# wwyuan2023/VITS

Hardware: AMD Instinct MI355X
Metric: 22.05 kHz audio samples/sec/GPU (infer RTF) + train utt/sec at 1/2/4/8 MI355X (higher is better)
Workload: dtype fp32; 1 GPU; SynthesizerTrn.infer_p2 batch=16 Tx=100 Ty=500 (configs/base.json, 16 kHz, hop 192) per GPU; global_batch=16, seq_len=500, parallelism=single GPU, graph=False

## Files before the change

### vits_amd/csrc/resblock_f32p.hip

```cpp
#include <type_traits>

#include "conv1d_impl.h"

namespace {

using vits_conv::fast_sigmoid;
using vits_conv::fast_tanh;
using vits_conv::split3_bf16x4;

constexpr int RP_GROUP = 3;
struct RpGroup {
  vits_resblock_pair_desc d[RP_GROUP];
  int n;
  int batch;
  int bn;
};

typedef __bf16 bf16x8 __attribute__((ext_vector_type(8)));
typedef __bf16 bf16x4 __attribute__((ext_vector_type(4)));
typedef __bf16 bf16x2 __attribute__((ext_vector_type(2)));
typedef float f32x4v __attribute__((ext_vector_type(4)));

template <int MODE>
struct RpT {
  typedef float xt;
  typedef __bf16 lt;
  static constexpr int NPL = 3;
};
template <>
struct RpT<1> {
  typedef __bf16 xt;
  typedef __bf16 lt;
  static constexpr int NPL = 1;
};
template <>
struct RpT<2> {
  typedef _Float16 xt;
  typedef _Float16 lt;
  static constexpr int NPL = 1;
};
__host__ __device__ constexpr int rp_npl(int mode) { return mode == 0 ? 3 : 1; }

__host__ __device__ constexpr int rp_ng(int C) { return C <= 64 ? 256 : 128; }
__host__ __device__ constexpr int rp_threads(int C) { return C == 256 ? 512 : 256; }
#ifndef VITS_RP_KC32
#define VITS_RP_KC32 32
#endif
__host__ __device__ constexpr int rp_kc(int C, int mode = 0) {
  return C == 256 ? 64 : C == 32 ? VITS_RP_KC32 : 16;
}
__host__ __device__ inline int rp_xcols(int NG, int k, int dil) {
  return ((NG + (k - 1) * dil + 3 + 3) >> 2) << 2;
}
__host__ __device__ inline int rp_lds_bytes(int C, int k, int dil, int mode = 0) {
  const int NG = rp_ng(C), npl = rp_npl(mode);
  const int nbuf = rp_kc(C, mode) < C ? 2 : 1;
  const int xs = nbuf * npl * rp_xcols(NG, k, dil) * (rp_kc(C, mode) + 4);
  const int gsz = npl * (NG + 16) * (C / 2 + 8);
  return 4 * 2 * C + 2 * (xs > gsz ? xs : gsz) + 64;
}
__host__ __device__ constexpr int rp_occ(int C, int) { return C == 256 ? 1 : 2; }

__device__ __forceinline__ float rp_gate(float a, float b) {
#pragma clang fp contract(off)
  return fast_tanh(a) * fast_sigmoid(b);
}

__device__ __forceinline__ float rp_max(float a, float b) {
  float r;
  asm("v_max_f32 %0, %1, %2" : "=v"(r) : "v"(a), "v"(b));
  return r;
}

template <int C, int MODE = 0, bool MEAN = false>
__global__ __launch_bounds__(rp_threads(C), rp_occ(C, MODE)) void resblock_f32p_kernel(
    const RpGroup G) {
  typedef std::integral_constant<bool, true> edge_t;
  typedef std::integral_constant<bool, false> interior_t;
  typedef typename RpT<MODE>::xt xt;
  typedef typename RpT<MODE>::lt lt;
  constexpr int NPL = RpT<MODE>::NPL;
  typedef lt lt8 __attribute__((ext_vector_type(8)));
  typedef lt lt4 __attribute__((ext_vector_type(4)));
  typedef lt lt2 __attribute__((ext_vector_type(2)));
  typedef xt xt4 __attribute__((ext_vector_type(4)));
  constexpr int H = C / 2;
  constexpr int NT = rp_threads(C);
  constexpr int WAVES_M = C >= 64 ? C / 64 : 1;
  constexpr int WAVES_N = NT / 64 / WAVES_M;
  constexpr int NG = 64 * WAVES_N;
  static_assert(NG == rp_ng(C), "tile columns");
  constexpr int TM = C >= 64 ? 2 : 1, TN = 2;
  constexpr int KC = rp_kc(C, MODE);
  constexpr int KCP = KC + 4;
  constexpr int GP = H + 8;
  constexpr int GPL = (NG + 16) * GP;
  constexpr int S1 = C / 16, S2 = H / 16;
  constexpr int NU = ((KC / 4) * ((NG + 102) / 4) + NT - 1) / NT;
  typedef lt8 av_t;
  constexpr int NB = NPL == 3 ? TN : 1;

  const int gi = MEAN ? 0 : (int)blockIdx.z / G.batch;
  const int b = (int)blockIdx.z - gi * G.batch;
  const int Tn = G.d[gi].t_len;
  const int L = G.d[gi].lengths ? min(Tn, (int)G.d[gi].lengths[b]) : Tn;
  const int BN = MEAN ? G.bn : NG - (G.d[gi].k - 1);
  const int n0 = blockIdx.x * BN;
  if (n0 >= Tn) return;
  if (G.d[gi].lengths && G.d[gi].len_skip > 0 && n0 >= L + G.d[gi].len_skip) return;

  extern __shared__ float smem[];
  float* const erow = smem;
  lt* const reg = reinterpret_cast<lt*>(smem + 2 * C);

  const int tid = threadIdx.x;
  const int lane = tid & 63;
  const int wid = __builtin_amdgcn_readfirstlane(tid >> 6);
  const int wn = (wid % WAVES_N) * 64;
  const int wm = (wid / WAVES_N) * 64;
  const int l32 = lane & 31;
  const int lhi = lane >> 5;

  float msum[TM][TN][MEAN ? 16 : 1];

#pragma unroll 1
  for (int br = 0; br < (MEAN ? G.n : 1); ++br) {
    const vits_resblock_pair_desc& p = G.d[MEAN ? br : gi];
    const int k = p.k;
    const int dil = p.dil;
    const int p1 = (k - 1) * dil / 2;
    const int p2 = (k - 1) / 2;
    const int tw0 = n0 - p2 - p1;
    const int xstart = tw0 & ~3;
    const int xcols = rp_xcols(NG, k, dil);
    const bool interior = xstart >= 0 && xstart + xcols <= Tn && n0 - p2 + NG <= L;
    if (MEAN && br > 0) __syncthreads();

    {
      const float* cond = p.cond ? p.cond + (int64_t)b * p.cond_bstride : nullptr;
      for (int r = tid; r < 2 * C; r += NT) {
        float e = 0.f;
        if (r < C) {
          const int idx = (r & 1) ? H + (r >> 1) : (r >> 1);
          if (p.b1) e = p.b1[idx];
          if (cond) e += cond[idx];
        } else if (p.b2) {
          e = p.b2[r - C];
        }
        erow[r] = e;
      }
    }

    f32x16 acc[TM][TN];
#pragma unroll
    for (int i = 0; i < TM; ++i)
#pragma unroll
      for (int j = 0; j < TN; ++j)
#pragma unroll
        for (int r = 0; r < 16; ++r) acc[i][j][r] = 0.f;

    auto mma = [&](av_t (*a)[TM], const av_t* bh, const av_t* bm, const av_t* bl) {
#pragma unroll
      for (int mi = 0; mi < TM; ++mi)
#pragma unroll
        for (int ni = 0; ni < TN; ++ni) {
          f32x16 c = acc[mi][ni];
          if constexpr (MODE == 0) {
            c = __builtin_amdgcn_mfma_f32_32x32x16_bf16(a[0][mi], bl[ni], c, 0, 0, 0);
            c = __builtin_amdgcn_mfma_f32_32x32x16_bf16(a[2][mi], bh[ni], c, 0, 0, 0);
            c = __builtin_amdgcn_mfma_f32_32x32x16_bf16(a[1][mi], bm[ni], c, 0, 0, 0);
            c = __builtin_amdgcn_mfma_f32_32x32x16_bf16(a[0][mi], bm[ni], c, 0, 0, 0);
            c = __builtin_amdgcn_mfma_f32_32x32x16_bf16(a[1][mi], bh[ni], c, 0, 0, 0);
            c = __builtin_amdgcn_mfma_f32_32x32x16_bf16(a[0][mi], bh[ni], c, 0, 0, 0);
          } else if constexpr (MODE == 1) {
            c = __builtin_amdgcn_mfma_f32_32x32x16_bf16(a[0][mi], bh[ni], c, 0, 0, 0);
          } else {
            c = __builtin_amdgcn_mfma_f32_32x32x16_f16(a[0][mi], bh[ni], c, 0, 0, 0);
          }
          acc[mi][ni] = c;
        }
    };
    auto loadA = [&](const lt* wl, int64_t wstep, int m_pad, int s, int total,
                     av_t (*a)[TM]) {
      const lt* wp = wl + (int64_t)(s < total ? s : total - 1) * wstep;
#pragma unroll
      for (int q = 0; q < NPL; ++q)
#pragma unroll
        for (int mi = 0; mi < TM; ++mi)
          a[q][mi] = *reinterpret_cast<const av_t*>(wp + ((int64_t)q * m_pad + mi * 32) * 8);
    };

    av_t a0[NPL][TM], a1[NPL][TM];
    av_t bh0[TN], bm0[NB], bl0[NB], bh1[TN], bm1[NB], bl1[NB];

    const xt* xb = reinterpret_cast<const xt*>(p.x) + (int64_t)b * p.x_bstride;
    {
      const int xsh = tw0 - xstart;
      const int nunits = (KC / 4) * (xcols >> 2);
      const int xpl = xcols * KCP;
      lt* const xbuf0 = reg;
      lt* const xbuf1 = reg + NPL * xpl;
      const float slope = p.in_slope;
      xt4 xr[NU][4];
      uint32_t xoff[NU];
      bool xok[NU];
#pragma unroll
      for (int q = 0; q < NU; ++q) {
        const int u = tid + NT * q;
        const int tt = xstart + 4 * (u / (KC / 4));
        xok[q] = u < nunits && tt >= 0 && tt < Tn;
        xoff[q] = xok[q] ? 4 * (u % (KC / 4)) * p.x_cstride + tt : 0;
      }
      auto gload = [&](int ch) __attribute__((always_inline)) {
        const xt* base = xb + (int64_t)ch * KC * p.x_cstride;
#pragma unroll
        for (int q = 0; q < NU; ++q) {
          if (q * NT < nunits) {
#pragma unroll
            for (int i = 0; i < 4; ++i)
              xr[q][i] = *reinterpret_cast<const xt4*>(base + (int64_t)i * p.x_cstride + xoff[q]);
          }
        }
      };
      const bool xfast = interior && slope > 0.f && slope < 1.f;
      auto lstore_as = [&](lt* xs, auto edge) __attribute__((always_inline)) {
#pragma unroll
        for (int q = 0; q < NU; ++q) {
          const int u = tid + NT * q;
          if (q * NT < nunits && u < nunits) {
            f32x4v v[4];
#pragma unroll
            for (int i = 0; i < 4; ++i)
#pragma unroll
              for (int e = 0; e < 4; ++e) {
                float t = (float)xr[q][i][e];
                if constexpr (decltype(edge)::value) {
                  t = t < 0.f ? t * slope : t;
                  v[i][e] = xok[q] ? t : 0.f;
                } else {
                  v[i][e] = rp_max(t, t * slope);
                }
              }
            lt* xh = xs + 4 * (u / (KC / 4)) * KCP + 4 * (u % (KC / 4));
#pragma unroll
            for (int e = 0; e < 4; ++e) {
              const f32x4v w = {v[0][e], v[1][e], v[2][e], v[3][e]};
              if constexpr (NPL == 3) {
                bf16x4 h4, m4, l4;
                split3_bf16x4(w, h4, m4, l4);
                *reinterpret_cast<bf16x4*>(xh + e * KCP) = h4;
                *reinterpret_cast<bf16x4*>(xh + xpl + e * KCP) = m4;
                *reinterpret_cast<bf16x4*>(xh + 2 * xpl + e * KCP) = l4;
              } else {
                lt4 w4;
#pragma unroll
                for (int i = 0; i < 4; ++i) w4[i] = (lt)w[i];
                *reinterpret_cast<lt4*>(xh + e * KCP) = w4;
              }
            }
          }
        }
      };
      auto lstore = [&](lt* xs) __attribute__((always_inline)) {
        if (xfast)
          lstore_as(xs, interior_t());
        else
          lstore_as(xs, edge_t());
      };
      auto loadB = [&](const lt* xs, int j, int g, av_t* bh, av_t* bm, av_t* bl) {
        const int P4 = xpl / 4;
#pragma unroll
        for (int ni = 0; ni < TN; ++ni) {
          const lt4* xp = reinterpret_cast<const lt4*>(
              xs + (wn + ni * 32 + l32 + j * dil + xsh) * KCP + 16 * g + 8 * lhi);
          bh[ni] = __builtin_shufflevector(xp[0], xp[1], 0, 1, 2, 3, 4, 5, 6, 7);
          if constexpr (NPL == 3) {
            bm[ni] = __builtin_shufflevector(xp[P4], xp[P4 + 1], 0, 1, 2, 3, 4, 5, 6, 7);
            bl[ni] = __builtin_shufflevector(xp[2 * P4], xp[2 * P4 + 1], 0, 1, 2, 3, 4, 5, 6, 7);
          }
        }
      };
      const lt* wl = reinterpret_cast<const lt*>(p.w1) +
                     ((int64_t)(lhi * NPL) * p.m_pad1 + wm + l32) * 8;
      const int64_t wstep = (int64_t)16 * NPL * p.m_pad1;
      const int total = S1 * k;
      const int nst = (KC / 16) * k;
      loadA(wl, wstep, p.m_pad1, 0, total, a0);
      gload(0);
      lstore(xbuf0);
      __syncthreads();
      for (int ch = 0; ch < C / KC; ++ch) {
        const bool more = ch + 1 < C / KC;
        if (more) gload(ch + 1);
        const lt* xs = (ch & 1) ? xbuf1 : xbuf0;
        const int s0 = ch * nst;
        int j = 0, g = 0;
        auto next = [&]() {
          if (++j == k) {
            j = 0;
            ++g;
          }
        };
        loadB(xs, 0, 0, bh0, bm0, bl0);
        int st = 0;
        for (; st + 2 <= nst; st += 2) {
          next();
          loadA(wl, wstep, p.m_pad1, s0 + st + 1, total, a1);
          loadB(xs, j, g, bh1, bm1, bl1);
          __builtin_amdgcn_sched_barrier(0);
          mma(a0, bh0, bm0, bl0);
          __builtin_amdgcn_sched_barrier(0);
          next();
          loadA(wl, wstep, p.m_pad1, s0 + st + 2, total, a0);
          if (st + 2 < nst) loadB(xs, j, g, bh0, bm0, bl0);
          __builtin_amdgcn_sched_barrier(0);
          mma(a1, bh1, bm1, bl1);
          __builtin_amdgcn_sched_barrier(0);
        }
        if (st < nst) {
          loadA(wl, wstep, p.m_pad1, s0 + nst, total, a1);
          __builtin_amdgcn_sched_barrier(0);
          mma(a0, bh0, bm0, bl0);
#pragma unroll
          for (int q = 0; q < NPL; ++q)
#pragma unroll
            for (int mi = 0; mi < TM; ++mi) a0[q][mi] = a1[q][mi];
        }
        if (more) lstore((ch & 1) ? xbuf0 : xbuf1);
        __syncthreads();
      }
    }

    lt* const gs = reg;
    auto gate = [&](auto edge) __attribute__((always_inline)) {
#pragma unroll
      for (int mi = 0; mi < TM; ++mi) {
        f32x4v er[4];
#pragma unroll
        for (int g = 0; g < 4; ++g)
          er[g] = *reinterpret_cast<const f32x4v*>(erow + wm + mi * 32 + 4 * lhi + 8 * g);
#pragma unroll
        for (int ni = 0; ni < TN; ++ni) {
          const int col = wn + ni * 32 + l32;
          const int t = n0 - p2 + col;
          const bool in = t >= 0 && t < L;
#pragma unroll
          for (int r = 0; r < 16; r += 4) {
            const int row = wm + mi * 32 + 4 * lhi + 8 * (r >> 2);
            const f32x4v e = er[r >> 2];
            float g0 = rp_gate(acc[mi][ni][r] + e[0], acc[mi][ni][r + 1] + e[1]);
            float g1 = rp_gate(acc[mi][ni][r + 2] + e[2], acc[mi][ni][r + 3] + e[3]);
            if constexpr (decltype(edge)::value) {
              g0 = in ? g0 : 0.f;
              g1 = in ? g1 : 0.f;
            }
            lt* gp = gs + col * GP + (row >> 1);
            if constexpr (NPL == 3) {
              const f32x4v w = {g0, g1, 0.f, 0.f};
              bf16x4 h4, m4, l4;
              split3_bf16x4(w, h4, m4, l4);
              *reinterpret_cast<bf16x2*>(gp) = __builtin_shufflevector(h4, h4, 0, 1);
              *reinterpret_cast<bf16x2*>(gp + GPL) = __builtin_shufflevector(m4, m4, 0, 1);
              *reinterpret_cast<bf16x2*>(gp + 2 * GPL) = __builtin_shufflevector(l4, l4, 0, 1);
            } else {
              lt2 v2;
              v2[0] = (lt)g0;
              v2[1] = (lt)g1;
              *reinterpret_cast<lt2*>(gp) = v2;
            }
          }
#pragma unroll
          for (int r = 0; r < 16; ++r) acc[mi][ni][r] = 0.f;
        }
      }
    };
    if (interior)
      gate(interior_t());
    else
      gate(edge_t());
    for (int i = tid; i < NPL * 16 * H; i += NT) {
      const int pl = i / (16 * H);
      const int e = i - pl * 16 * H;
      gs[pl * GPL + (NG + e / H) * GP + e % H] = (lt)0.f;
    }
    __syncthreads();

    {
      const lt* wl = reinterpret_cast<const lt*>(p.w2) +
                     ((int64_t)(lhi * NPL) * p.m_pad2 + wm + l32) * 8;
      const int64_t wstep = (int64_t)16 * NPL * p.m_pad2;
      const int total = S2 * k;
      const lt* gl = gs + (wn + l32) * GP + 8 * lhi;
      int j = 0, g = 0;
      auto loadB = [&](av_t* bh, av_t* bm, av_t* bl) {
        const lt* x = gl + j * GP + 16 * g;
#pragma unroll
        for (int ni = 0; ni < TN; ++ni) {
          bh[ni] = *reinterpret_cast<const av_t*>(x + ni * 32 * GP);
          if constexpr (NPL == 3) {
            bm[ni] = *reinterpret_cast<const av_t*>(x + ni * 32 * GP + GPL);
            bl[ni] = *reinterpret_cast<const av_t*>(x + ni * 32 * GP + 2 * GPL);
          }
        }
        if (++j == k) {
          j = 0;
          ++g;
        }
      };
      loadA(wl, wstep, p.m_pad2, 0, total, a0);
      loadB(bh0, bm0, bl0);
      int s = 0;
      for (; s + 2 <= total; s += 2) {
        loadA(wl, wstep, p.m_pad2, s + 1, total, a1);
        loadB(bh1, bm1, bl1);
        __builtin_amdgcn_sched_barrier(0);
        mma(a0, bh0, bm0, bl0);
        __builtin_amdgcn_sched_barrier(0);
        loadA(wl, wstep, p.m_pad2, s + 2, total, a0);
        if (s + 2 < total) loadB(bh0, bm0, bl0);
        __builtin_amdgcn_sched_barrier(0);
        mma(a1, bh1, bm1, bl1);
        __builtin_amdgcn_sched_barrier(0);
      }
      if (s < total) mma(a0, bh0, bm0, bl0);
    }

    xt* const yb = reinterpret_cast<xt*>(p.y) + (int64_t)b * p.y_bstride;
    const bool accum = !MEAN && p.accumulate;
    const float div = MEAN ? (float)G.n : p.post_div;
    const bool last = !MEAN || br == G.n - 1;
    auto epilogue = [&](auto edge) __attribute__((always_inline)) {
#pragma unroll
      for (int mi = 0; mi < TM; ++mi) {
        const xt* const xrow = xb + (int64_t)(wm + mi * 32) * p.x_cstride;
        xt* const yrow = yb + (int64_t)(wm + mi * 32) * p.y_cstride;
        f32x4v e2[4];
#pragma unroll
        for (int g = 0; g < 4; ++g)
          e2[g] = *reinterpret_cast<const f32x4v*>(erow + C + wm + mi * 32 + 4 * lhi + 8 * g);
#pragma unroll
        for (int ni = 0; ni < TN; ++ni) {
          const int col = wn + ni * 32 + l32;
          const int t = n0 + col;
          const bool st = decltype(edge)::value ? col < BN && t < Tn : col < BN;
          const int tc = st ? t : 0;
          const uint32_t xv = (uint32_t)(4 * lhi * p.x_cstride + tc) * (uint32_t)sizeof(xt);
          const uint32_t yv = (uint32_t)(4 * lhi * p.y_cstride + tc) * (uint32_t)sizeof(xt);
          auto xat = [&](int r) __attribute__((always_inline)) -> const xt& {
            const xt* row = xrow + (int64_t)((r & 3) + 8 * (r >> 2)) * p.x_cstride;
            return *reinterpret_cast<const xt*>(reinterpret_cast<const char*>(row) + xv);
          };
          auto yat = [&](int r) __attribute__((always_inline)) -> xt& {
            xt* row = yrow + (int64_t)((r & 3) + 8 * (r >> 2)) * p.y_cstride;
            return *reinterpret_cast<xt*>(reinterpret_cast<char*>(row) + yv);
          };
          float o[16];
#pragma unroll
          for (int r = 0; r < 16; ++r) {
            const float rv = (float)xat(r);
            const float v = acc[mi][ni][r] + e2[r >> 2][r & 3];
            o[r] = rv + v;
          }
          if constexpr (MEAN) {
#pragma unroll
            for (int r = 0; r < 16; ++r) {
              o[r] = br == 0 ? o[r] : msum[mi][ni][r] + o[r];
              msum[mi][ni][r] = o[r];
            }
          }
          if (accum) {
#pragma unroll
            for (int r = 0; r < 16; ++r)
              o[r] = (float)yat(r) + o[r];
          }
          if (last) {
            if (div != 1.0f) {
#pragma unroll
              for (int r = 0; r < 16; ++r) o[r] = o[r] / div;
            }
            if (st) {
#pragma unroll
              for (int r = 0; r < 16; ++r) {
                if constexpr (decltype(edge)::value) o[r] = t < L ? o[r] : 0.f;
                yat(r) = (xt)o[r];
              }
            }
          }
        }
      }
    };
    if (interior)
      epilogue(interior_t());
    else
      epilogue(edge_t());
  }
}

template <int C, int MODE = 0, bool MEAN = false>
int rp_launch(const RpGroup& g, hipStream_t s) {
  int lds = 0, gx = 0;
  for (int i = 0; i < g.n; ++i) {
    const vits_resblock_pair_desc& d = g.d[i];
    const int l = rp_lds_bytes(C, d.k, d.dil, MODE);
    if (l > lds) lds = l;
    const int BN = MEAN ? g.bn : rp_ng(C) - (d.k - 1);
    const int x = (d.t_len + BN - 1) / BN;
    if (x > gx) gx = x;
  }
  if (lds > 160 * 1024) return VITS_E_UNSUP;
  hipLaunchKernelGGL((resblock_f32p_kernel<C, MODE, MEAN>),
                     dim3(gx, 1, MEAN ? g.batch : g.n * g.batch), dim3(rp_threads(C)), lds, s, g);
  return vits_launch_status();
}

int rp_check(const vits_resblock_pair_desc& d, int mode = 0) {
  VITS_CHECK_ARG(d.x && d.w1 && d.w2 && d.y);
  VITS_CHECK_ARG(reinterpret_cast<const void*>(d.y) != reinterpret_cast<const void*>(d.x));
  VITS_CHECK_SHAPE(d.channels == 32 || d.channels == 64 || d.channels == 128 ||
                   d.channels == 256);
  VITS_CHECK_SHAPE(d.k >= 1 && d.k <= 15 && (d.k & 1) == 1 && d.dil >= 1 && d.t_len > 0);
  VITS_CHECK_SHAPE((d.k - 1) * d.dil <= 96);
  VITS_CHECK_SHAPE(d.m_pad1 >= d.channels && d.m_pad2 >= d.channels && (d.m_pad1 & 3) == 0 &&
                   (d.m_pad2 & 3) == 0);
  VITS_CHECK_SHAPE(d.cin_pad1 >= d.channels && d.cin_pad2 >= d.channels / 2);
  VITS_CHECK_SHAPE((d.t_len & 3) == 0 && (d.x_cstride & 3) == 0 && (d.x_bstride & 3) == 0 &&
                   d.x_cstride >= d.t_len && d.y_cstride >= d.t_len &&
                   (reinterpret_cast<uintptr_t>(d.x) & (mode ? 7 : 15)) == 0);
  VITS_CHECK_SHAPE((int64_t)d.channels * d.x_cstride < (1LL << 31));
  VITS_CHECK_SHAPE((int64_t)d.channels * d.y_cstride < (1LL << 31));
  VITS_CHECK_SHAPE((reinterpret_cast<uintptr_t>(d.w1) & 15) == 0 &&
                   (reinterpret_cast<uintptr_t>(d.w2) & 15) == 0);
  return VITS_OK;
}

}

int vits_rp16_256(const vits_resblock_pair_desc* d, int n, int batch, int wdtype,
                  hipStream_t s) {
  if (!d || n < 1 || n > RP_GROUP || batch < 1) return VITS_E_ARG;
  if (wdtype != VITS_WDT_BF16 && wdtype != VITS_WDT_F16) return VITS_E_ARG;
  const int mode = wdtype == VITS_WDT_BF16 ? 1 : 2;
  RpGroup g;
  g.n = n;
  g.batch = batch;
  g.bn = 0;
  for (int i = 0; i < n; ++i) {
    const int rc = rp_check(d[i], mode);
    if (rc) return rc;
    if (d[i].channels != d[0].channels) return VITS_E_SHAPE;
    g.d[i] = d[i];
  }
  if (d[0].channels != 256) return VITS_E_SHAPE;
  return mode == 1 ? rp_launch<256, 1>(g, s) : rp_launch<256, 2>(g, s);
}

extern "C" int vits_resblock_pair_f32p_forward(const vits_resblock_pair_desc* d, int n, int batch,
                                               void* stream) {
  if (!d || n < 1 || n > RP_GROUP || batch < 1) return VITS_E_ARG;
  RpGroup g;
  g.n = n;
  g.batch = batch;
  g.bn = 0;
  for (int i = 0; i < n; ++i) {
    const int rc = rp_check(d[i]);
    if (rc) return rc;
    if (d[i].channels != d[0].channels) return VITS_E_SHAPE;
    g.d[i] = d[i];
  }
  hipStream_t s = as_stream(stream);
  int rc;
  if (d[0].channels == 32)
    rc = rp_launch<32>(g, s);
  else if (d[0].channels == 64)
    rc = rp_launch<64>(g, s);
  else if (d[0].channels == 128)
    rc = rp_launch<128>(g, s);
  else
    rc = rp_launch<256>(g, s);
  return count_ok(rc, VITS_CNT_RESBLOCK);
}

extern "C" int vits_resblock_pair_f32p_mean_forward(const vits_resblock_pair_desc* d, int n,
                                                    int batch, void* stream) {
  if (!d || n < 1 || n > RP_GROUP || batch < 1) return VITS_E_ARG;
  RpGroup g;
  g.n = n;
  g.batch = batch;
  int kmax = 1;
  for (int i = 0; i < n; ++i) {
    const int rc = rp_check(d[i]);
    if (rc) return rc;
    VITS_CHECK_SHAPE(d[i].channels == 32);
    VITS_CHECK_SHAPE(d[i].t_len == d[0].t_len && d[i].lengths == d[0].lengths &&
                     d[i].len_skip == d[0].len_skip && d[i].y == d[0].y &&
                     d[i].y_bstride == d[0].y_bstride && d[i].y_cstride == d[0].y_cstride);
    VITS_CHECK_ARG(reinterpret_cast<const void*>(d[0].y) != reinterpret_cast<const void*>(d[i].x));
    if (d[i].k > kmax) kmax = d[i].k;
    g.d[i] = d[i];
  }
  g.bn = rp_ng(32) - (kmax - 1);
  return count_ok(rp_launch<32, 0, true>(g, as_stream(stream)), VITS_CNT_RESBLOCK);
}
```

### vits_amd/ops.py

```python
from __future__ import annotations

import contextlib
import ctypes as C
import math
import threading
from dataclasses import dataclass, field
from fractions import Fraction
from typing import Optional

import numpy as np
import torch

from . import _lib
from ._lib import (ACT_NONE, WDT_BF16, WDT_F16, WDT_F32, WDT_F32P, WDT_F32S, ConvDesc, ConvOut, EPI_GATE, EPI_STORE,
                   ResblockPairDesc,
                   EPI_UPSAMPLE, TILE_128x128, TILE_32x256, TILE_64x128, TILE_64x256, TILE_ROWS,
                   check)



def _stream_ptr(device: torch.device) -> int:
    return torch.cuda.current_stream(device).cuda_stream


# ... 179 lines not shown
    m = (r.view(torch.int32) & mask).view(torch.float32)
    lo = r - m
    return torch.stack([h, m, lo], dim=-3).to(torch.bfloat16)


F32S_MIN_ROWS = 0


def _f32s_min_rows() -> int:
    return F32S_MIN_ROWS or (64 if SPLIT_W else 128)


def to_lowp(layer: PackedConv, wdtype: int = WDT_BF16, min_rows: Optional[int] = None) -> PackedConv:
    if layer.wdtype != WDT_F32 or wdtype == WDT_F32:
        return layer
    if wdtype == WDT_F32S:
        if layer.m < (_f32s_min_rows() if min_rows is None else min_rows):
            return layer
        kc = 16
        w32 = layer.w[:layer.cin]
        cin_pad = (layer.cin + kc - 1) // kc * kc
        k, m_pad = w32.shape[1], w32.shape[2]
        w = w32.new_zeros(cin_pad, k, m_pad)
        w[:layer.cin] = w32
        w = w.view(cin_pad // kc, kc // 8, 8, k, m_pad).permute(0, 3, 1, 4, 2).contiguous()
        if SPLIT_W:
            tile = _pick_tile_f32p(layer.m, layer.k)
            return PackedConv(split_planes(w), layer.bias, layer.cin, layer.m, layer.k,
                              layer.dil, layer.pad_left, layer.epi, tile,
                              _kc_f32p(cin_pad, layer.k, layer.dil, tile), up_u=layer.up_u,
                              up_pad=layer.up_pad, out_channels=layer.out_channels,
                              extra=layer.extra, wdtype=WDT_F32P)
        return PackedConv(w, layer.bias, layer.cin, layer.m, layer.k, layer.dil,
                          layer.pad_left, layer.epi, _pick_tile_f32s(layer.m, layer.k), kc,
                          up_u=layer.up_u, up_pad=layer.up_pad,
                          out_channels=layer.out_channels, extra=layer.extra, wdtype=wdtype)
    kc = 16
    w32 = layer.w[:layer.cin]
    cin_pad = (layer.cin + kc - 1) // kc * kc
    k, m_pad = w32.shape[1], w32.shape[2]
    w = w32.new_zeros(cin_pad, k, m_pad)
    w[:layer.cin] = w32
    w = w.view(cin_pad // kc, kc // 8, 8, k, m_pad).permute(0, 3, 1, 4, 2).contiguous()
    tile = _pick_tile_bf16(layer.m, layer.k)
    return PackedConv(w.to(_WDT_TORCH[wdtype]), layer.bias, layer.cin, layer.m, layer.k,
                      layer.dil, layer.pad_left, layer.epi, tile, kc, up_u=layer.up_u,
                      up_pad=layer.up_pad, out_channels=layer.out_channels, extra=layer.extra,
                      wdtype=wdtype)


LOWP_KCK = 512


def io16_kc(layer: PackedConv) -> int:
    bm, bn = TILE_ROWS[layer.tile], TILE_COLS[layer.tile]
    xrs = bn + (layer.k - 1) * layer.dil + 8
    xbudget = 6144 if bn <= 128 else 10240
    for kc in (64, 48, 32):
        if (kc * layer.k <= LOWP_KCK and layer.cin_pad % kc == 0
                and kc * layer.k * bm // 2 <= 6144 and kc * xrs <= xbudget):
            return kc
    return 16


def to_bf16(layer: PackedConv) -> PackedConv:
    return to_lowp(layer, WDT_BF16)


def pack_conv(weight: torch.Tensor, bias: Optional[torch.Tensor], *, dilation: int = 1,
              padding: Optional[int] = None, gate: bool = False) -> PackedConv:
    w = weight.detach().to(torch.float32)
    cout, cin, k = w.shape
    if padding is None:
        padding = (k * dilation - dilation) // 2
    if gate:
        assert cout % 2 == 0
        h = cout // 2
        rows = torch.stack([w[:h], w[h:]], dim=1).reshape(cout, cin, k)
        epi, outc = EPI_GATE, h
    else:
        rows, epi, outc = w, EPI_STORE, cout
    tile = _pick_tile(cout, k)
    packed, kc = _finish_pack(rows, k, tile, dilation)
    b = None if bias is None else bias.detach().to(torch.float32).contiguous()
    layer = PackedConv(packed, b, cin, cout, k, dilation, padding, epi, tile, kc,
                       out_channels=outc)
    return to_lowp(layer, PACK_PRECISION.wdtype)


def pack_conv_transpose(weight: torch.Tensor, bias: Optional[torch.Tensor], stride: int,
                        padding: int) -> PackedConv:
    w = weight.detach().to(torch.float32)
    cin, cout, K = w.shape
    u = stride
    assert K % u == 0, "polyphase lowering needs kernel_size % stride == 0"
    kp = K // u
    w4 = w.reshape(cin, cout, kp, u)
    rows = w4.flip(2).permute(1, 3, 0, 2).reshape(cout * u, cin, kp)
    tile = _pick_tile(cout * u, kp)
    packed, kc = _finish_pack(rows, kp, tile)
    b = None if bias is None else bias.detach().to(torch.float32).contiguous()
    layer = PackedConv(packed, b, cin, cout * u, kp, 1, kp - 1, EPI_UPSAMPLE, tile, kc,
                       up_u=u, up_pad=padding, out_channels=cout)
    return to_lowp(layer, PACK_PRECISION.wdtype)




def make_out(y: torch.Tensor, *, act: int = ACT_NONE, res: Optional[torch.Tensor] = None,
             res_scale: float = 1.0, accumulate: bool = False, post_div: float = 1.0,
             channel_offset: int = 0) -> ConvOut:
    o = ConvOut()
    o.y = y.data_ptr() + y.element_size() * channel_offset * y.stride(1)
    o.y_bstride = y.stride(0)
    o.y_cstride = y.stride(1)
    o.act = act
    if res is not None:
        o.res = res.data_ptr() + res.element_size() * channel_offset * res.stride(1)
        o.res_bstride = res.stride(0)
        o.res_cstride = res.stride(1)
    else:
        o.res = None
        o.res_bstride = 0
        o.res_cstride = 0
    o.res_scale = res_scale
    o.accumulate = 1 if accumulate else 0
    o.post_div = post_div
    return o


_LOWP_TORCH = {WDT_F16: torch.float16, WDT_BF16: torch.bfloat16}


class _LenSkip(threading.local):
    margin = 0


LEN_SKIP = _LenSkip()


@contextlib.contextmanager
def length_skip(margin: int = 64):
    old = LEN_SKIP.margin
    LEN_SKIP.margin = int(margin)
    try:
        yield
    finally:
        LEN_SKIP.margin = old


def make_desc(layer: PackedConv, x: torch.Tensor, out0: ConvOut, *, out1: Optional[ConvOut] = None,
              split: Optional[int] = None, tin: Optional[int] = None, n_out: Optional[int] = None,
              in_slope: float = 1.0, cond: Optional[torch.Tensor] = None, cond_offset: int = 0,
              lengths: Optional[torch.Tensor] = None, t_out: int = 0,
              x_channel_offset: int = 0, io16: bool = False) -> ConvDesc:
    if io16:
        assert layer.wdtype != WDT_F32 and x.dtype == _LOWP_TORCH[layer.wdtype]
    else:
        assert x.dtype == torch.float32
    d = ConvDesc()
    d.x = x.data_ptr() + x.element_size() * x_channel_offset * x.stride(1)
    d.io16 = int(io16)
    d.x_bstride = x.stride(0)
    d.x_cstride = x.stride(1)
    d.x_tstride = x.stride(2)
    d.cin = layer.cin
    d.tin = x.shape[2] if tin is None else tin
    d.in_slope = in_slope
    d.w = layer.w.data_ptr()
    d.m = layer.m
    d.m_pad = layer.m_pad
    d.cin_pad = layer.cin_pad
    d.kc = layer.kc
    d.k = layer.k
    d.dil = layer.dil
    d.pad_left = layer.pad_left
    if n_out is None:
        if layer.epi == EPI_UPSAMPLE:
            n_out = d.tin + (layer.up_pad + layer.up_u - 1) // layer.up_u
        else:
            n_out = d.tin
    d.n_out = n_out
    d.tile = layer.tile
    d.epi = layer.epi
    d.bias = _ptr(layer.bias)
    if cond is not None:
        d.cond = cond.data_ptr() + 4 * cond_offset
        d.cond_bstride = cond.stride(0)
    else:
        d.cond = None
        d.cond_bstride = 0
    d.split = layer.m if split is None else split
    d.up_u = layer.up_u
    d.up_pad = layer.up_pad
    d.t_out = t_out
    d.lengths = _ptr(lengths)
    d.len_skip = LEN_SKIP.margin if lengths is not None else 0
    d.out0 = out0
    if out1 is not None:
        d.out1 = out1
    d.wdtype = layer.wdtype
    return d


def conv_flops(desc: ConvDesc, batch: int) -> int:
    cols = desc.tin if desc.epi == EPI_UPSAMPLE else desc.n_out
    return 2 * batch * desc.m * cols * desc.cin * desc.k


BF16_DENSE_PEAK_TFLOPS = 2500.0
MFMA_PEAK_TFLOPS = {WDT_F32: 157.3, WDT_BF16: BF16_DENSE_PEAK_TFLOPS,
                    WDT_F16: BF16_DENSE_PEAK_TFLOPS, WDT_F32S: BF16_DENSE_PEAK_TFLOPS / 6,
                    WDT_F32P: BF16_DENSE_PEAK_TFLOPS / 6}


class ConvTimer:

    active = None

    def __init__(self):
        self.records = []
        self.shapes = []
        self.peaks = []

    def __enter__(self):
        ConvTimer.active = self
        return self

    def __exit__(self, *exc):
        ConvTimer.active = None
        return False

    def launch(self, lib, desc, batch, device):
        group = tuple(desc) if isinstance(desc, (tuple, list)) else (desc,)
        s = torch.cuda.Event(enable_timing=True)
        e = torch.cuda.Event(enable_timing=True)
        stream = torch.cuda.current_stream(device)
        s.record(stream)
        arr = (ConvDesc * len(group))(*group)
        sizes = (C.c_int32 * 1)(len(group))
        check(lib.vits_conv1d_forward_groups(arr, sizes, 1, batch, stream.cuda_stream),
              "vits_conv1d_forward_groups")
        e.record(stream)
        self.records.append((s, e, sum(conv_flops(d, batch) for d in group)))
        self.peaks.append(MFMA_PEAK_TFLOPS[group[0].wdtype])
        self.shapes.append("conv " + "+".join(
            f"m{d.m}c{d.cin}k{d.k}d{d.dil}T{d.n_out}e{d.epi}t{d.tile}" for d in group))

    def launch_pairs(self, lib, group, batch, device, wdtype=None, mean=False):
        s = torch.cuda.Event(enable_timing=True)
        e = torch.cuda.Event(enable_timing=True)
        stream = torch.cuda.current_stream(device)
        s.record(stream)
        arr = (ResblockPairDesc * len(group))(*group)
        if wdtype is None:
            check(lib.vits_resblock_pair_forward(arr, len(group), batch, stream.cuda_stream),
                  "vits_resblock_pair_forward")
        elif wdtype == WDT_F32P:
            fn = (lib.vits_resblock_pair_f32p_mean_forward if mean
                  else lib.vits_resblock_pair_f32p_forward)
            check(fn(arr, len(group), batch, stream.cuda_stream),
                  "vits_resblock_pair_f32p_forward")
        else:
            fn = lib.vits_resblock_pair16_mean_forward if mean else lib.vits_resblock_pair16_forward
            check(fn(arr, len(group), batch, int(wdtype), stream.cuda_stream),
                  "vits_resblock_pair16_forward")
        e.record(stream)
        self.records.append((s, e, sum(resblock_pair_flops(d, batch) for d in group)))
        self.peaks.append(MFMA_PEAK_TFLOPS[WDT_F32 if wdtype is None else
                                           WDT_F32S if wdtype == WDT_F32P else wdtype])
        self.shapes.append("pair " + "+".join(
            f"C{d.channels}k{d.k}d{d.dil}T{d.t_len}" for d in group))

    def summary(self):
        torch.cuda.synchronize()
        ms = [s.elapsed_time(e) for s, e, _ in self.records]
        fl = [f for _, _, f in self.records]
        min_ms = sum(f / (pk * 1e9) for f, pk in zip(fl, self.peaks))
        return dict(launches=len(ms), total_ms=float(sum(ms)), total_flops=int(sum(fl)),
                    avg_ms=float(sum(ms) / max(1, len(ms))), mfma_bound_ms=float(min_ms),
                    f32s_flops=int(sum(f for f, pk in zip(fl, self.peaks)
                                       if pk == MFMA_PEAK_TFLOPS[WDT_F32S])))

    def per_launch(self):
        torch.cuda.synchronize()
        return [(lab, s.elapsed_time(e), f)
                for lab, (s, e, f) in zip(self.shapes, self.records)]


_RB_KC = {}


RESBLOCK_PAIR_MAX_K = 7


def resblock_pair_supported(c1: PackedConv, c2: PackedConv, T: int) -> bool:
    C = c2.out_channels
    return (c1.wdtype == WDT_F32 and c2.wdtype == WDT_F32 and C in (32, 64)
            and c1.m == C and c1.cin == C and c2.cin == C // 2 and c1.k == c2.k
            and c1.k <= RESBLOCK_PAIR_MAX_K and c2.dil == 1 and T % 4 == 0
            and _resblock_kc(C, c1.k, c1.dil) is not None)


F32P_PAIR_MAX_K = {32: 11, 64: 11, 128: 7, 256: 3}


def resblock_pair_f32p_supported(c1: PackedConv, c2: PackedConv, x: torch.Tensor) -> bool:
    C_ = c2.out_channels
    return (c1.wdtype == WDT_F32P and c2.wdtype == WDT_F32P and c1.k <= F32P_PAIR_MAX_K.get(C_, 0)
            and x.dtype == torch.float32 and c1.m == C_ and c1.cin == C_ and c2.cin == C_ // 2
            and c2.m == C_ and c1.k == c2.k and c1.k % 2 == 1 and (c1.k - 1) * c1.dil <= 96
            and c2.dil == 1 and c1.epi == EPI_GATE and c2.epi == EPI_STORE
            and (C_ != 256 or (c1.k - 1) * c1.dil <= 56)
            and c1.pad_left == (c1.k - 1) * c1.dil // 2 and c2.pad_left == (c2.k - 1) // 2
            and x.shape[2] % 4 == 0 and x.stride(2) == 1 and x.stride(1) % 4 == 0
            and x.stride(0) % 4 == 0 and x.data_ptr() % 16 == 0)


def _resblock_kc(ch: int, k: int, dil: int):
    key = (ch, k, dil)
    if key not in _RB_KC:
        kc1, kc2 = C.c_int(), C.c_int()
        rc = _lib.load().vits_resblock_pair_kc(ch, k, dil, kc1, kc2)
        _RB_KC[key] = (kc1.value, kc2.value) if rc == 0 else None
    return _RB_KC[key]


def resblock_pair_desc(c1: PackedConv, c2: PackedConv, x: torch.Tensor, y: torch.Tensor, *,
                       cond: Optional[torch.Tensor] = None, cond_offset: int = 0,
                       in_slope: float = 0.1, accumulate: bool = False,
                       post_div: float = 1.0,
                       lengths: Optional[torch.Tensor] = None) -> ResblockPairDesc:
    assert x.dtype == torch.float32 and y.dtype == torch.float32 and x.stride(2) == 1
    C_, T = x.shape[1], x.shape[2]
    kc1, kc2 = (16, 16) if c1.wdtype == WDT_F32P else _resblock_kc(C_, c1.k, c1.dil)
    d = ResblockPairDesc()
    d.x, d.x_bstride, d.x_cstride, d.t_len = x.data_ptr(), x.stride(0), x.stride(1), T
    d.channels, d.in_slope = C_, in_slope
    d.w1, d.m_pad1, d.cin_pad1, d.kc1 = c1.w.data_ptr(), c1.m_pad, c1.cin_pad, kc1
    d.k, d.dil, d.kc2 = c1.k, c1.dil, kc2
    d.b1 = _ptr(c1.bias)
    if cond is not None:
        d.cond, d.cond_bstride = cond.data_ptr() + 4 * cond_offset, cond.stride(0)
    d.w2, d.m_pad2, d.cin_pad2 = c2.w.data_ptr(), c2.m_pad, c2.cin_pad
    d.b2 = _ptr(c2.bias)
    d.y, d.y_bstride, d.y_cstride = y.data_ptr(), y.stride(0), y.stride(1)
    d.accumulate, d.post_div = int(accumulate), float(post_div)
    d.lengths = _ptr(lengths)
    d.len_skip = LEN_SKIP.margin if lengths is not None else 0
    return d


FUSED_PAIRS16 = True
PAIR16_256_MAX_K = 15


def resblock_pair16_supported(c1: PackedConv, c2: PackedConv, x: torch.Tensor) -> bool:
    C_ = c2.out_channels
    if C_ == 256 and c1.k > PAIR16_256_MAX_K:
        return False
    return (FUSED_PAIRS16 and c1.wdtype in (WDT_BF16, WDT_F16) and c2.wdtype == c1.wdtype
            and x.dtype == _WDT_TORCH[c1.wdtype] and C_ in (32, 64, 128, 256) and c1.m == C_
            and c1.cin == C_ and c2.cin == C_ // 2 and c2.m == C_ and c1.k == c2.k
            and c1.k % 2 == 1 and (c1.k - 1) * c1.dil <= 96 and c2.dil == 1
            and c1.epi == EPI_GATE and x.shape[2] % 4 == 0 and x.stride(2) == 1
            and x.stride(1) % 4 == 0 and x.stride(0) % 4 == 0)


def resblock_pair16_desc(c1: PackedConv, c2: PackedConv, x: torch.Tensor, y: torch.Tensor, *,
                         cond: Optional[torch.Tensor] = None, cond_offset: int = 0,
                         in_slope: float = 0.1, accumulate: bool = False, post_div: float = 1.0,
                         lengths: Optional[torch.Tensor] = None) -> ResblockPairDesc:
    assert x.dtype == y.dtype == _WDT_TORCH[c1.wdtype] and x.stride(2) == 1 and y.stride(2) == 1
    C_, T = x.shape[1], x.shape[2]
    d = ResblockPairDesc()
    d.x, d.x_bstride, d.x_cstride, d.t_len = x.data_ptr(), x.stride(0), x.stride(1), T
    d.channels, d.in_slope = C_, in_slope
    d.w1, d.m_pad1, d.cin_pad1, d.kc1 = c1.w.data_ptr(), c1.m_pad, c1.cin_pad, 16
    d.k, d.dil, d.kc2 = c1.k, c1.dil, 16
    d.b1 = _ptr(c1.bias)
    if cond is not None:
        d.cond, d.cond_bstride = cond.data_ptr() + 4 * cond_offset, cond.stride(0)
    d.w2, d.m_pad2, d.cin_pad2 = c2.w.data_ptr(), c2.m_pad, c2.cin_pad
    d.b2 = _ptr(c2.bias)
    d.y, d.y_bstride, d.y_cstride = y.data_ptr(), y.stride(0), y.stride(1)
    d.accumulate, d.post_div = int(accumulate), float(post_div)
    d.lengths = _ptr(lengths)
    d.len_skip = LEN_SKIP.margin if lengths is not None else 0
    return d


def resblock_pair16_launch(descs, batch: int, device: torch.device, wdtype: int,
                           mean: bool = False):
    group = tuple(descs) if isinstance(descs, (tuple, list)) else (descs,)
    lib = _lib.load()
    if ConvTimer.active is not None:
        return ConvTimer.active.launch_pairs(lib, group, batch, device, wdtype, mean=mean)
    arr = (ResblockPairDesc * len(group))(*group)
    fn = lib.vits_resblock_pair16_mean_forward if mean else lib.vits_resblock_pair16_forward
    check(fn(arr, len(group), batch, int(wdtype), _stream_ptr(device)),
          "vits_resblock_pair16_forward")


def resblock_pair_flops(d: ResblockPairDesc, batch: int) -> int:
    C_, k, T = d.channels, d.k, d.t_len
    return 2 * batch * T * (C_ * C_ * k + (C_ // 2) * C_ * k)


def resblock_pair_launch(descs, batch: int, device: torch.device, wdtype: int = WDT_F32,
                         mean: bool = False):
    group = tuple(descs) if isinstance(descs, (tuple, list)) else (descs,)
    lib = _lib.load()
    if mean and wdtype != WDT_F32P:
        raise NotImplementedError("branch-mean launch: split-fp32 pairs only")
    if ConvTimer.active is not None:
        return ConvTimer.active.launch_pairs(lib, group, batch, device,
                                             wdtype=WDT_F32P if wdtype == WDT_F32P else None,
                                             mean=mean)
    arr = (ResblockPairDesc * len(group))(*group)
    if wdtype == WDT_F32P:
        fn = (lib.vits_resblock_pair_f32p_mean_forward if mean
              else lib.vits_resblock_pair_f32p_forward)
        check(fn(arr, len(group), batch, _stream_ptr(device)), "vits_resblock_pair_f32p_forward")
        return
    check(lib.vits_resblock_pair_forward(arr, len(group), batch, _stream_ptr(device)),
          "vits_resblock_pair_forward")


def conv1d_launch(desc: ConvDesc, batch: int, device: torch.device):
    lib = _lib.load()
    if ConvTimer.active is not None:
        return ConvTimer.active.launch(lib, desc, batch, device)
    check(lib.vits_conv1d_forward(C.byref(desc), batch, _stream_ptr(device)), "vits_conv1d_forward")


def conv1d_launch_seq(descs, batch: int, device: torch.device):
    lib = _lib.load()
    if ConvTimer.active is not None:
        for d in descs:
            ConvTimer.active.launch(lib, d, batch, device)
        return
    flat, sizes = [], []
    for d in descs:
        group = tuple(d) if isinstance(d, (tuple, list)) else (d,)
        flat.extend(group)
        sizes.append(len(group))
    arr = (ConvDesc * len(flat))(*flat)
    sz = (C.c_int32 * len(sizes))(*sizes)
    check(lib.vits_conv1d_forward_groups(arr, sz, len(sizes), batch, _stream_ptr(device)),
          "vits_conv1d_forward_groups")


def conv1d(x: torch.Tensor, layer: PackedConv, *, in_slope: float = 1.0, act: int = ACT_NONE,
           cond: Optional[torch.Tensor] = None, residual: Optional[torch.Tensor] = None,
           res_scale: float = 1.0, lengths: Optional[torch.Tensor] = None,
           out: Optional[torch.Tensor] = None, accumulate: bool = False,
           post_div: float = 1.0, t_out: Optional[int] = None) -> torch.Tensor:
    require_device(x, cond, residual, lengths)
    B, _, T = x.shape
    io16 = x.dtype != torch.float32
    if layer.epi == EPI_UPSAMPLE:
        T_out = T * layer.up_u if t_out is None else t_out
    else:
        T_out = T
    if out is None:
        out = torch.empty(B, layer.out_channels, T_out, device=x.device, dtype=x.dtype)
    o0 = make_out(out, act=act, res=residual, res_scale=res_scale, accumulate=accumulate,
                  post_div=post_div)
    if lengths is not None:
        lengths = lengths.to(device=x.device, dtype=torch.int32).contiguous()
    d = make_desc(layer, x, o0, in_slope=in_slope, cond=cond, lengths=lengths, t_out=T_out,
                  io16=2 if io16 else 0)
    conv1d_launch(d, B, x.device)
    return out




def linear_rows(g: torch.Tensor, weight: torch.Tensor, bias: Optional[torch.Tensor],
                out: Optional[torch.Tensor] = None) -> torch.Tensor:
    require_device(g, weight, bias)
    g = g.contiguous().float()
    B, n_in = g.shape
    n_out = weight.shape[0]
    if out is None:
        out = torch.empty(B, n_out, device=g.device, dtype=torch.float32)
    lib = _lib.load()
    check(lib.vits_linear_forward(g.data_ptr(), g.stride(0), weight.data_ptr(), _ptr(bias),
                                  out.data_ptr(), out.stride(0), B, n_out, n_in,
                                  _stream_ptr(g.device)), "vits_linear_forward")
    return out


def expand_prior(attn: torch.Tensor, m_p: torch.Tensor, s_p: torch.Tensor, noise: torch.Tensor,
                 out: Optional[torch.Tensor] = None, exp_s: bool = False,
                 noise_scale: float = 1.0) -> torch.Tensor:
    require_device(attn, m_p, s_p, noise)
    attn = attn.contiguous().float()
    m_p = m_p.contiguous().float()
    s_p = s_p.contiguous().float()
    noise = noise.contiguous().float()
    B, Ty, Tx = attn.shape
    Cc = m_p.shape[1]
    if out is None:
        out = torch.empty(B, Cc, Ty, device=attn.device, dtype=torch.float32)
    lib = _lib.load()
    check(lib.vits_expand_prior(attn.data_ptr(), m_p.data_ptr(), s_p.data_ptr(), noise.data_ptr(),
                                out.data_ptr(), B, Cc, Ty, Tx, 1 if exp_s else 0, noise_scale,
                                _stream_ptr(attn.device)),
          "vits_expand_prior")
    return out


ED_DRAWS = 32


def numpy_draw_pool(n: int = ED_DRAWS):
    state = np.random.get_state()
    words = np.random.randint(0, 2 ** 32, size=n, dtype=np.uint32)
    return words.view(np.int32).copy(), state


def numpy_draw_commit(state, used: int) -> None:
    np.random.set_state(state)
    if used > 0:
        np.random.randint(0, 2 ** 32, size=used, dtype=np.uint32)


def expand_durations(logw: torch.Tensor, m_p: torch.Tensor, s_p: torch.Tensor,
                     noise: torch.Tensor, t_y: int, *, rate: float = 1.0,
                     noise_scale: float = 1.0, x_len: Optional[torch.Tensor] = None,
                     noise_start: Optional[torch.Tensor] = None, half_round: bool = False,
                     stage_mult=(1,), out: Optional[torch.Tensor] = None,
                     lens: Optional[torch.Tensor] = None,
                     starts: Optional[torch.Tensor] = None):
    require_device(logw, m_p, s_p, noise)
    if starts is not None:
        if noise_start is not None:
            raise _lib.VitsAmdError("expand_durations: give noise_start or starts, not both")
        require_device(starts)
        if (tuple(starts.shape) != (m_p.shape[0],) or starts.dtype != torch.int64
                or not starts.is_contiguous()):
            raise _lib.VitsAmdError(f"expand_durations: starts must be int64 [{m_p.shape[0]}]")
    B, C_, t_x = m_p.shape
    logw = logw.reshape(B, t_x).float().contiguous()
    m_p = m_p.float().contiguous()
    s_p = s_p.float().contiguous()
    noise = noise.float().contiguous()
    if out is None:
        out = torch.empty(B, C_, t_y, device=m_p.device, dtype=torch.float32)
    n_stage = len(stage_mult)
    rows = n_stage + (0 if noise_start is None else 1)
    if lens is None:
        lens = torch.empty(rows, B, device=m_p.device, dtype=torch.int32)
    if tuple(lens.shape) != (rows, B) or lens.dtype != torch.int32 or not lens.is_contiguous():
        raise _lib.VitsAmdError(f"expand_durations: lens must be int32 [{rows}, {B}]")
    mult = (C.c_int32 * n_stage)(*[int(v) for v in stage_mult])
    if starts is not None:
        mode, start_ptr = 2, starts.data_ptr()
    elif noise_start is None:
        assert tuple(noise.shape) == (B, C_, t_y), noise.shape
        mode, start_ptr = 0, None
    elif (tuple(noise_start.shape) != (B, ED_DRAWS) or noise_start.dtype != torch.int32
          or not noise_start.is_contiguous()):
        raise _lib.VitsAmdError(f"expand_durations: noise_start must be int32 [{B}, {ED_DRAWS}]")
    else:
        mode, start_ptr = 1, noise_start.data_ptr()
    check(_lib.load().vits_expand_durations(
        logw.data_ptr(), logw.stride(0), _ptr(x_len), t_x, float(rate), int(half_round),
        m_p.data_ptr(), s_p.data_ptr(), m_p.stride(0), m_p.stride(1), noise.data_ptr(),
        mode, start_ptr, noise.numel(), float(noise_scale),
        out.data_ptr(),
        B, C_, t_y, lens.data_ptr(), mult, n_stage, _stream_ptr(m_p.device)),
        "vits_expand_durations")
    return out, lens


def _n_rows_ptr(n_rows, B: int, device, what: str):
    if n_rows is None:
        return None, None
    if not isinstance(n_rows, torch.Tensor):
        if not 0 <= int(n_rows) <= B:
            raise _lib.VitsAmdError(f"{what}: n_rows must be in [0, {B}], got {n_rows}")
        n_rows = torch.tensor([int(n_rows)], dtype=torch.int32, device=device)
    require_device(n_rows)
    if n_rows.dtype != torch.int32 or n_rows.numel() != 1:
        raise _lib.VitsAmdError(f"{what}: n_rows must be an int or an int32 [1] device tensor")
    return n_rows, n_rows.data_ptr()


def draw_starts(logw: torch.Tensor, channels: int, noise_len: int, pool: torch.Tensor, *,
                rate: float = 1.0, x_len: Optional[torch.Tensor] = None,
                half_round: bool = False, n_rows=None, starts: Optional[torch.Tensor] = None,
                meta: Optional[torch.Tensor] = None):
    require_device(logw, pool)
    B = logw.shape[0]
    logw = logw.reshape(B, -1).float().contiguous()
    t_x = logw.shape[1]
    if pool.dtype != torch.int32 or pool.dim() != 1 or not pool.is_contiguous() or not pool.numel():
        raise _lib.VitsAmdError("draw_starts: pool must be a contiguous int32 [P] tensor, P >= 1")
    if starts is None:
        starts = torch.empty(B, device=logw.device, dtype=torch.int64)
    if meta is None:
        meta = torch.empty(2 * B + 1, device=logw.device, dtype=torch.int32)
    if (tuple(starts.shape) != (B,) or starts.dtype != torch.int64 or not starts.is_contiguous()
            or tuple(meta.shape) != (2 * B + 1,) or meta.dtype != torch.int32
            or not meta.is_contiguous()):
# ... 471 lines not shown
```

Measured before the change: 78.34 million output samples/s.

## Use single-row wave tiles with more waves and rematerialized addressing in resblock kernel

```diff
diff --git a/vits_amd/csrc/resblock_f32p.hip b/vits_amd/csrc/resblock_f32p.hip
--- a/vits_amd/csrc/resblock_f32p.hip
+++ b/vits_amd/csrc/resblock_f32p.hip
@@ -42,7 +42,30 @@
 __host__ __device__ constexpr int rp_npl(int mode) { return mode == 0 ? 3 : 1; }
 
 __host__ __device__ constexpr int rp_ng(int C) { return C <= 64 ? 256 : 128; }
-__host__ __device__ constexpr int rp_threads(int C) { return C == 256 ? 512 : 256; }
+#ifndef VITS_RP_TM64
+#define VITS_RP_TM64 1
+#endif
+#ifndef VITS_RP_TM128
+#define VITS_RP_TM128 1
+#endif
+#ifndef VITS_RP_TM256
+#define VITS_RP_TM256 1
+#endif
+#ifdef VITS_RP_OTHER_SIDE
+#define VITS_RP_SIDE(tm) (3 - (tm))
+#else
+#define VITS_RP_SIDE(tm) (tm)
+#endif
+__host__ __device__ constexpr int rp_tm(int C, int mode = 0) {
+  return C == 32     ? 1
+         : mode != 0 ? 2
+         : C == 64   ? VITS_RP_SIDE(VITS_RP_TM64)
+         : C == 128  ? VITS_RP_SIDE(VITS_RP_TM128)
+                     : VITS_RP_SIDE(VITS_RP_TM256);
+}
+__host__ __device__ constexpr int rp_threads(int C, int tm) {
+  return (C / (32 * tm)) * (rp_ng(C) / 64) * 64;
+}
 #ifndef VITS_RP_KC32
 #define VITS_RP_KC32 32
 #endif
@@ -59,7 +82,9 @@
   const int gsz = npl * (NG + 16) * (C / 2 + 8);
   return 4 * 2 * C + 2 * (xs > gsz ? xs : gsz) + 64;
 }
-__host__ __device__ constexpr int rp_occ(int C, int) { return C == 256 ? 1 : 2; }
+__host__ __device__ constexpr int rp_occ(int C, int, int tm) {
+  return tm == 1 && C >= 64 ? 4 : C == 256 ? 1 : 2;
+}
 
 __device__ __forceinline__ float rp_gate(float a, float b) {
 #pragma clang fp contract(off)
@@ -72,8 +97,21 @@
   return r;
 }
 
-template <int C, int MODE = 0, bool MEAN = false>
-__global__ __launch_bounds__(rp_threads(C), rp_occ(C, MODE)) void resblock_f32p_kernel(
+template <typename T>
+__device__ __forceinline__ T rp_fresh(T v) {
+  asm volatile("" : "+v"(v));
+  return v;
+}
+
+template <typename T>
+__device__ __forceinline__ const T* rp_sbase(const T* p) {
+  uint64_t u = reinterpret_cast<uint64_t>(p);
+  asm("" : "+s"(u));
+  return (const T*)reinterpret_cast<const __attribute__((address_space(1))) T*>(u);
+}
+
+template <int C, int MODE = 0, bool MEAN = false, int TM = rp_tm(C, MODE)>
+__global__ __launch_bounds__(rp_threads(C, TM), rp_occ(C, MODE, TM)) void resblock_f32p_kernel(
     const RpGroup G) {
   typedef std::integral_constant<bool, true> edge_t;
   typedef std::integral_constant<bool, false> interior_t;
@@ -85,12 +123,13 @@
   typedef lt lt2 __attribute__((ext_vector_type(2)));
   typedef xt xt4 __attribute__((ext_vector_type(4)));
   constexpr int H = C / 2;
-  constexpr int NT = rp_threads(C);
-  constexpr int WAVES_M = C >= 64 ? C / 64 : 1;
+  static_assert(TM == 1 || (TM == 2 && C >= 64), "wave tile rows");
+  constexpr int NT = rp_threads(C, TM);
+  constexpr int WAVES_M = C / (32 * TM);
   constexpr int WAVES_N = NT / 64 / WAVES_M;
   constexpr int NG = 64 * WAVES_N;
   static_assert(NG == rp_ng(C), "tile columns");
-  constexpr int TM = C >= 64 ? 2 : 1, TN = 2;
+  constexpr int TN = 2;
   constexpr int KC = rp_kc(C, MODE);
   constexpr int KCP = KC + 4;
   constexpr int GP = H + 8;
@@ -99,6 +138,7 @@
   constexpr int NU = ((KC / 4) * ((NG + 102) / 4) + NT - 1) / NT;
   typedef lt8 av_t;
   constexpr int NB = NPL == 3 ? TN : 1;
+  constexpr bool REMAT = TM == 1 && C >= 64;
 
   const int gi = MEAN ? 0 : (int)blockIdx.z / G.batch;
   const int b = (int)blockIdx.z - gi * G.batch;
@@ -117,7 +157,7 @@
   const int lane = tid & 63;
   const int wid = __builtin_amdgcn_readfirstlane(tid >> 6);
   const int wn = (wid % WAVES_N) * 64;
-  const int wm = (wid / WAVES_N) * 64;
+  const int wm = (wid / WAVES_N) * (32 * TM);
   const int l32 = lane & 31;
   const int lhi = lane >> 5;
 
@@ -180,14 +220,21 @@
           acc[mi][ni] = c;
         }
     };
-    auto loadA = [&](const lt* wl, int64_t wstep, int m_pad, int s, int total,
+    auto loadA = [&](const lt* w, uint32_t al, int64_t wstep, int m_pad, int s, int total,
                      av_t (*a)[TM]) {
-      const lt* wp = wl + (int64_t)(s < total ? s : total - 1) * wstep;
+      const lt* wp = w + (int64_t)(s < total ? s : total - 1) * wstep + (int64_t)wm * 8;
+      const uint32_t av = REMAT ? rp_fresh(al) : al;
 #pragma unroll
       for (int q = 0; q < NPL; ++q)
 #pragma unroll
         for (int mi = 0; mi < TM; ++mi)
-          a[q][mi] = *reinterpret_cast<const av_t*>(wp + ((int64_t)q * m_pad + mi * 32) * 8);
+          if constexpr (REMAT)
+            a[q][mi] = *reinterpret_cast<const av_t*>(
+                reinterpret_cast<const char*>(rp_sbase(wp + ((int64_t)q * m_pad + mi * 32) * 8)) +
+                av);
+          else
+            a[q][mi] = *reinterpret_cast<const av_t*>(
+                reinterpret_cast<const char*>(wp + ((int64_t)q * m_pad + mi * 32) * 8) + av);
     };
 
     av_t a0[NPL][TM], a1[NPL][TM];
@@ -201,6 +248,8 @@
       lt* const xbuf0 = reg;
       lt* const xbuf1 = reg + NPL * xpl;
       const float slope = p.in_slope;
+      constexpr bool XB = KC * sizeof(xt) <= 2 * C;
+      constexpr uint32_t XU = XB ? (uint32_t)sizeof(xt) : 1u;
       xt4 xr[NU][4];
       uint32_t xoff[NU];
       bool xok[NU];
@@ -209,24 +258,30 @@
         const int u = tid + NT * q;
         const int tt = xstart + 4 * (u / (KC / 4));
         xok[q] = u < nunits && tt >= 0 && tt < Tn;
-        xoff[q] = xok[q] ? 4 * (u % (KC / 4)) * p.x_cstride + tt : 0;
+        xoff[q] = xok[q] ? (uint32_t)(4 * (u % (KC / 4)) * p.x_cstride + tt) * XU : 0;
       }
       auto gload = [&](int ch) __attribute__((always_inline)) {
         const xt* base = xb + (int64_t)ch * KC * p.x_cstride;
 #pragma unroll
         for (int q = 0; q < NU; ++q) {
           if (q * NT < nunits) {
-#pragma unroll
-            for (int i = 0; i < 4; ++i)
-              xr[q][i] = *reinterpret_cast<const xt4*>(base + (int64_t)i * p.x_cstride + xoff[q]);
+            const uint32_t xo = REMAT ? rp_fresh(xoff[q]) : xoff[q];
+#pragma unroll
+            for (int i = 0; i < 4; ++i) {
+              const xt* row = base + (int64_t)i * p.x_cstride;
+              if constexpr (REMAT) row = rp_sbase(row);
+              xr[q][i] = *reinterpret_cast<const xt4*>(reinterpret_cast<const char*>(row) +
+                                                       (size_t)xo * (sizeof(xt) / XU));
+            }
           }
         }
       };
       const bool xfast = interior && slope > 0.f && slope < 1.f;
       auto lstore_as = [&](lt* xs, auto edge) __attribute__((always_inline)) {
+        const int ftid = REMAT ? rp_fresh(tid) : tid;
 #pragma unroll
         for (int q = 0; q < NU; ++q) {
-          const int u = tid + NT * q;
+          const int u = ftid + NT * q;
           if (q * NT < nunits && u < nunits) {
             f32x4v v[4];
 #pragma unroll
@@ -280,12 +335,12 @@
           }
         }
       };
-      const lt* wl = reinterpret_cast<const lt*>(p.w1) +
-                     ((int64_t)(lhi * NPL) * p.m_pad1 + wm + l32) * 8;
+      const lt* wl = reinterpret_cast<const lt*>(p.w1);
+      const uint32_t al = (uint32_t)((lhi * NPL) * p.m_pad1 + l32) * (uint32_t)(8 * sizeof(lt));
       const int64_t wstep = (int64_t)16 * NPL * p.m_pad1;
       const int total = S1 * k;
       const int nst = (KC / 16) * k;
-      loadA(wl, wstep, p.m_pad1, 0, total, a0);
+      loadA(wl, al, wstep, p.m_pad1, 0, total, a0);
       gload(0);
       lstore(xbuf0);
       __syncthreads();
@@ -305,20 +360,20 @@
         int st = 0;
         for (; st + 2 <= nst; st += 2) {
           next();
-          loadA(wl, wstep, p.m_pad1, s0 + st + 1, total, a1);
+          loadA(wl, al, wstep, p.m_pad1, s0 + st + 1, total, a1);
           loadB(xs, j, g, bh1, bm1, bl1);
           __builtin_amdgcn_sched_barrier(0);
           mma(a0, bh0, bm0, bl0);
           __builtin_amdgcn_sched_barrier(0);
           next();
-          loadA(wl, wstep, p.m_pad1, s0 + st + 2, total, a0);
+          loadA(wl, al, wstep, p.m_pad1, s0 + st + 2, total, a0);
           if (st + 2 < nst) loadB(xs, j, g, bh0, bm0, bl0);
           __builtin_amdgcn_sched_barrier(0);
           mma(a1, bh1, bm1, bl1);
           __builtin_amdgcn_sched_barrier(0);
         }
         if (st < nst) {
-          loadA(wl, wstep, p.m_pad1, s0 + nst, total, a1);
+          loadA(wl, al, wstep, p.m_pad1, s0 + nst, total, a1);
           __builtin_amdgcn_sched_barrier(0);
           mma(a0, bh0, bm0, bl0);
 #pragma unroll
@@ -333,6 +388,8 @@
 
     lt* const gs = reg;
     auto gate = [&](auto edge) __attribute__((always_inline)) {
+      const int flane = REMAT ? rp_fresh(lane) : lane;
+      const int l32 = flane & 31, lhi = flane >> 5;
 #pragma unroll
       for (int mi = 0; mi < TM; ++mi) {
         f32x4v er[4];
@@ -386,8 +443,10 @@
     __syncthreads();
 
     {
-      const lt* wl = reinterpret_cast<const lt*>(p.w2) +
-                     ((int64_t)(lhi * NPL) * p.m_pad2 + wm + l32) * 8;
+      const int flane = REMAT ? rp_fresh(lane) : lane;
+      const int l32 = flane & 31, lhi = flane >> 5;
+      const lt* wl = reinterpret_cast<const lt*>(p.w2);
+      const uint32_t al = (uint32_t)((lhi * NPL) * p.m_pad2 + l32) * (uint32_t)(8 * sizeof(lt));
       const int64_t wstep = (int64_t)16 * NPL * p.m_pad2;
       const int total = S2 * k;
       const lt* gl = gs + (wn + l32) * GP + 8 * lhi;
@@ -407,16 +466,16 @@
           ++g;
         }
       };
-      loadA(wl, wstep, p.m_pad2, 0, total, a0);
+      loadA(wl, al, wstep, p.m_pad2, 0, total, a0);
       loadB(bh0, bm0, bl0);
       int s = 0;
       for (; s + 2 <= total; s += 2) {
-        loadA(wl, wstep, p.m_pad2, s + 1, total, a1);
+        loadA(wl, al, wstep, p.m_pad2, s + 1, total, a1);
         loadB(bh1, bm1, bl1);
         __builtin_amdgcn_sched_barrier(0);
         mma(a0, bh0, bm0, bl0);
         __builtin_amdgcn_sched_barrier(0);
-        loadA(wl, wstep, p.m_pad2, s + 2, total, a0);
+        loadA(wl, al, wstep, p.m_pad2, s + 2, total, a0);
         if (s + 2 < total) loadB(bh0, bm0, bl0);
         __builtin_amdgcn_sched_barrier(0);
         mma(a1, bh1, bm1, bl1);
@@ -430,6 +489,8 @@
     const float div = MEAN ? (float)G.n : p.post_div;
     const bool last = !MEAN || br == G.n - 1;
     auto epilogue = [&](auto edge) __attribute__((always_inline)) {
+      const int flane = REMAT ? rp_fresh(lane) : lane;
+      const int l32 = flane & 31, lhi = flane >> 5;
 #pragma unroll
       for (int mi = 0; mi < TM; ++mi) {
         const xt* const xrow = xb + (int64_t)(wm + mi * 32) * p.x_cstride;
@@ -496,7 +557,7 @@
   }
 }
 
-template <int C, int MODE = 0, bool MEAN = false>
+template <int C, int MODE = 0, bool MEAN = false, int TM = rp_tm(C, MODE)>
 int rp_launch(const RpGroup& g, hipStream_t s) {
   int lds = 0, gx = 0;
   for (int i = 0; i < g.n; ++i) {
@@ -508,8 +569,9 @@
     if (x > gx) gx = x;
   }
   if (lds > 160 * 1024) return VITS_E_UNSUP;
-  hipLaunchKernelGGL((resblock_f32p_kernel<C, MODE, MEAN>),
-                     dim3(gx, 1, MEAN ? g.batch : g.n * g.batch), dim3(rp_threads(C)), lds, s, g);
+  hipLaunchKernelGGL((resblock_f32p_kernel<C, MODE, MEAN, TM>),
+                     dim3(gx, 1, MEAN ? g.batch : g.n * g.batch), dim3(rp_threads(C, TM)), lds, s,
+                     g);
   return vits_launch_status();
 }
 
diff --git a/vits_amd/ops.py b/vits_amd/ops.py
--- a/vits_amd/ops.py
+++ b/vits_amd/ops.py
@@ -505,7 +505,7 @@
             and _resblock_kc(C, c1.k, c1.dil) is not None)
 
 
-F32P_PAIR_MAX_K = {32: 11, 64: 11, 128: 7, 256: 3}
+F32P_PAIR_MAX_K = {32: 11, 64: 11, 128: 11, 256: 3}
 
 
 def resblock_pair_f32p_supported(c1: PackedConv, c2: PackedConv, x: torch.Tensor) -> bool:
```

Measured after the change: 80.09 million output samples/s, median of 6. 2.2% higher.
